# RIKEN-RCCS/EigenExa

Hardware: AMD Instinct MI355X
Metric: eigen_sx full-solve throughput (reference flop model: 4/3 N^3 + D&C GEMM + 2 nvec N^2) (higher is better)
Workload: dtype f64; 1 GPU; N=8192 random symmetric fp64 (counter-based R+R^T, seed 20240807), eigen_sx all eigenpairs, m_forward=64, m_backward=128; parallelism=1 GPU (1x1 grid)

## Files before the change

### eigenexa_amd/csrc/api.hip

```cpp
#include "eigx_context.h"
#include "eigx_comm.h"
#include "../../include/eigenexa_amd.h"
#include <cstring>

namespace eigx {
Context g_ctx;
}

using namespace eigx;

extern "C" {

int eigx_init(int device) {
  return eigx_init_multi(device, 0, 1, nullptr, 'C');
}

int eigx_get_device_count(void) {
  int ndev = 0;
  if (hipGetDeviceCount(&ndev) != hipSuccess) { (void)hipGetLastError(); return 0; }
  return ndev;
}

int eigx_get_rccl_unique_id(void* out128) {
  return comm_get_unique_id(out128);
// ... 160 lines not shown
  const int Px = x_procs, Py = y_procs;
  const int mb = m_backward > 0 ? m_backward : 128;
  const int n1 = ceil_div(n, Px);
  const int n2 = ceil_div(n, Py);
  int lnx;
  int64_t lny;
  if (mode == 'M' || mode == 'm') {
    lnx = n1; lny = n2;
  } else if (mode == 'L' || mode == 'l') {
    lnx = ceil_div(n1, 32) * 32; lny = n2;
  } else {
    lnx = ceil_div(n1, 64) * 64 + 32;
    if (lnx < n1 + 64) lnx += 64;
    const int NB = mb > 64 ? mb : 64;
    int64_t nmz = (int64_t)ceil_div(n1, NB) * NB + 1;
    const int64_t nmz2 = (int64_t)ceil_div(ceil_div(n, NB), Px) * NB;
    if (nmz2 > nmz) nmz = nmz2;
    int64_t nmw = (int64_t)ceil_div(n2, NB) * NB + 1;
    const int64_t nmw2 = (int64_t)ceil_div(ceil_div(n, NB), Py) * NB;
    if (nmw2 > nmw) nmw = nmw2;
    nmz += NB; nmw += NB;
    const int64_t big = nmz > lnx ? nmz : lnx;
    lny = ceil_div64(big * nmw, lnx);
    if (lny < n2) lny = n2;
    lnx = hbm_ld(lnx);
  }
  {
    const int P = Px * Py;
    const int nf = ceil_div(n, P);
    const int64_t nx0 = (int64_t)nf * (P / Px), ny0 = (int64_t)nf * (P / Py);
    if (nx0 > lnx) lnx = (int)nx0;
    if (ny0 > lny) lny = ny0;
  }
  const int pmin = Px < Py ? Px : Py;
  const int64_t side = ceil_div64(ceil_div(n, pmin), 64) * 64;
  if ((side * side >= ((int64_t)1 << 31) || lny >= ((int64_t)1 << 31)) && !(getenv("EIGX_ALLOW_64BIT"))) {
    *nx = -1; *ny = -1;
    return EIGX_ERR_TOO_LARGE;
  }
  *nx = lnx;
  *ny = (int)lny;
  return EIGX_OK;
}

int eigx_get_matdims(int n, int* nx, int* ny, int m_forward, int m_backward, char mode) {
  if (!g_ctx.initialized) return EIGX_ERR_NOT_INITIALIZED;
  return eigx_matdims_for_grid(n, g_ctx.grid.Px, g_ctx.grid.Py, m_forward, m_backward, mode, nx, ny);
}

int64_t eigx_memory_internal(int n, int lda, int ldz, int m_forward, int m_backward) {
  if (!g_ctx.initialized) return -1;
  return solver_workspace_bytes(g_ctx, n, lda, ldz, m_forward, m_backward);
}

int64_t eigx_held_bytes(void) {
  if (!g_ctx.initialized) return -1;
  int64_t t = 0;
  for (const auto& kv : g_ctx.pool.bufs) t += (int64_t)kv.second.bytes;
  return t + comm_held_bytes(g_ctx);
}

int64_t eigx_held_bytes_named(const char* prefix) {
  if (!g_ctx.initialized || !prefix) return -1;
  const std::string pre(prefix);
  int64_t t = 0;
  for (const auto& kv : g_ctx.pool.bufs)
    if (kv.first.compare(0, pre.size(), pre) == 0) t += (int64_t)kv.second.bytes;
  return t;
}

int eigx_get_timers(double* out16) {
  if (!out16) return EIGX_ERR_BAD_ARG;
  for (int i = 0; i < 16; ++i) out16[i] = g_ctx.timers[i];
  return EIGX_OK;
}

int eigx_profile(int stride) {
  if (!g_ctx.initialized) return EIGX_ERR_NOT_INITIALIZED;
  g_ctx.prof_stride = stride > 0 ? stride : 0;
  g_ctx.prof_used = 0;
  g_ctx.prof_kind.clear();
  g_ctx.prof_units.clear();
  return EIGX_OK;
}

int eigx_profile_read(double* out6) {
  if (!g_ctx.initialized) return EIGX_ERR_NOT_INITIALIZED;
  if (!out6) return EIGX_ERR_BAD_ARG;
  EIGX_HIP_CHECK(hipSetDevice(g_ctx.device));
  EIGX_HIP_CHECK(hipStreamSynchronize(g_ctx.stream));
  for (int q = 0; q < 6; ++q) out6[q] = 0.0;
  for (size_t q = 0; q < g_ctx.prof_kind.size(); ++q) {
    float ms = 0.f;
    EIGX_HIP_CHECK(hipEventElapsedTime(&ms, g_ctx.prof_ev[2 * q], g_ctx.prof_ev[2 * q + 1]));
    if (g_ctx.prof_kind[q] > 1) continue;
    const int k = g_ctx.prof_kind[q] ? 3 : 0;
    out6[k + 0] += 1.0;
    out6[k + 1] += g_ctx.prof_units[q];
    out6[k + 2] += 1e-3 * ms;
  }
  return EIGX_OK;
}

int eigx_profile_read_kinds(double* out, int nkinds) {
  if (!g_ctx.initialized) return EIGX_ERR_NOT_INITIALIZED;
  if (!out || nkinds < 1) return EIGX_ERR_BAD_ARG;
  EIGX_HIP_CHECK(hipSetDevice(g_ctx.device));
  EIGX_HIP_CHECK(hipStreamSynchronize(g_ctx.stream));
  for (int q = 0; q < 3 * nkinds; ++q) out[q] = 0.0;
  for (size_t q = 0; q < g_ctx.prof_kind.size(); ++q) {
    const int k = g_ctx.prof_kind[q];
    if (k < 0 || k >= nkinds) continue;
    float ms = 0.f;
    EIGX_HIP_CHECK(hipEventElapsedTime(&ms, g_ctx.prof_ev[2 * q], g_ctx.prof_ev[2 * q + 1]));
    out[3 * k + 0] += 1.0;
    out[3 * k + 1] += g_ctx.prof_units[q];
    out[3 * k + 2] += 1e-3 * ms;
  }
  return EIGX_OK;
}

int eigx_device_synchronize(void) {
  if (!g_ctx.initialized) return EIGX_ERR_NOT_INITIALIZED;
  EIGX_HIP_CHECK(hipSetDevice(g_ctx.device));
  EIGX_HIP_CHECK(hipDeviceSynchronize());
  return EIGX_OK;
}

void* eigx_malloc_dev(int64_t bytes) {
  if (!g_ctx.initialized) return nullptr;
  void* p = nullptr;
  if (hipMalloc(&p, (size_t)bytes) != hipSuccess) return nullptr;
  return p;
}
int eigx_free_dev(void* p) {
  if (p) EIGX_HIP_CHECK(hipFree(p));
  return EIGX_OK;
}
int eigx_memcpy_h2d(void* dst, const void* src, int64_t bytes) {
  EIGX_HIP_CHECK(hipMemcpy(dst, src, (size_t)bytes, hipMemcpyHostToDevice));
  return EIGX_OK;
}
int eigx_memcpy_d2h(void* dst, const void* src, int64_t bytes) {
  EIGX_HIP_CHECK(hipMemcpy(dst, src, (size_t)bytes, hipMemcpyDeviceToHost));
  return EIGX_OK;
}

int eigx_tune(int key, int value) {
  if (key == 0) return set_gemm_variant(value);
  if (key == 1) return set_bisect_threads(value);
  if (key == 2) return set_bt_q(value);
  if (key == 3 || key == 4 || key == 5 || key == 10 || key == 11) return set_reduce_knob(key, value);
  if (key == 12) return (value >= 0 && value <= 2) ? set_reduce_knob(key, value) : -1;
  if (key == 6) return set_gemm_cstream(value);
  if (key == 7) return value > 0 ? set_reduce_knob(key, value) : -1;
  if (key == 8) return set_dc_chunk(value);
  if (key == 9) return comm_set_bounce(value);
  if (key == 15) return set_dc_pipe(value);
  if (key == 16) return set_dc_batch(value);
  if (key == 17 || key == 18 || key == 19) return set_range_knob(key, value);
  if (key == 20) return set_tri_nb(value);
  if (key == 21) return set_batch_nmax(value);
  if (key == 22) return set_hbatch_nmax(value);
  if (key == 23) return set_gbatch_nmax(value);
  if (key == 24) return set_hgbatch_nmax(value);
  if (key == 25) return set_gemm_latec_kmax(value);
  if (key == 26) return set_batch_range_route(value);
  if (key == 27) return set_batch_range_accept(value);
  return -1;
}

int eigx_dgemm_dev(char opa, char opb, int m, int n, int k, double alpha, const double* a, int lda,
                   const double* b, int ldb, double beta, double* c, int ldc, int tri_upper) {
  if (!g_ctx.initialized) return EIGX_ERR_NOT_INITIALIZED;
  EIGX_HIP_CHECK(hipStreamSynchronize(nullptr));
  dgemm_dev(g_ctx.stream, opa, opb, m, n, k, alpha, a, lda, b, ldb, beta, c, ldc, tri_upper ? 1 : 0,
            &g_ctx.grid);
  EIGX_HIP_CHECK(hipStreamSynchronize(g_ctx.stream));
  return EIGX_OK;
}

int eigx_dgemm_gather_dev(char opa, char opb, int m, int n, int k, double alpha, const double* a, int lda,
                          const double* b, int ldb, double beta, double* c, int ldc, const int* kmap_a,
                          const int* kmap_b) {
  if (!g_ctx.initialized) return EIGX_ERR_NOT_INITIALIZED;
  EIGX_HIP_CHECK(hipStreamSynchronize(nullptr));
  dgemm_dev(g_ctx.stream, opa, opb, m, n, k, alpha, a, lda, b, ldb, beta, c, ldc, 0, nullptr, kmap_a, nullptr, 1, 0,
            0, 0, 1, 0, 0, 0, 1, 0, kmap_b);
  EIGX_HIP_CHECK(hipStreamSynchronize(g_ctx.stream));
  return EIGX_OK;
}

}
```

### eigenexa_amd/csrc/band_reduce.hip

```cpp
#include "eigx_context.h"
#include "eigx_comm.h"
#include "../../include/eigenexa_amd.h"
#include <algorithm>
#include <chrono>
#include <cstring>
#include <type_traits>

#pragma clang fp contract(on)

namespace eigx {

namespace {

static inline int pd_rows_for(int toprows) { int r = ((toprows + 3) / 4 + 63) / 64 * 64; return r < 512 ? 512 : r; }
#ifdef EIGX_STAMPS
#define EIGX_ABL(bit) (R.abl & (bit))
#define EIGX_STAMP(slot) do { if (R.dbg && threadIdx.x == 0 && stamp_me) { \
  const unsigned long long _t = __builtin_amdgcn_s_memtime(); atomicAdd(&R.dbg[slot], _t - stamp_prev); stamp_prev = _t; } } while (0)
#define EIGX_STAMP_INIT const bool stamp_me = (bid == nblocks / 2); unsigned long long stamp_prev = __builtin_amdgcn_s_memtime(); (void)stamp_me;
#else
#define EIGX_ABL(bit) false
#define EIGX_STAMP(slot) do {} while (0)
#define EIGX_STAMP_INIT
#endif
constexpr int PD_COLS = 16;
constexpr int KA_ROWS = 16;
constexpr int KA_SL = 256 / KA_ROWS;

enum { SC_SA = 0, SC_BETA_A = 1, SC_SB = 2, SC_BETA_B = 3, SC_COUNT = 8 };

struct RedArgs {
  double* A; int lda; int n;
  double* UW; int ldp; int m;
  double* X;
  double* YR; double* YC;
  double* KD;
  double* SP;
  int sp_packed;
  int kd_compact;
  double* GP;
  double* sc;
  double* d; double* e; int lde;
  int maxseg, maxrs, maxchunk, gp2_off, kdab_off;
  int P, me;
  float invP;
  int Px, Py, px, py, row_major;
  int nxs, nys;
  const double* MSG;
  int msg_stride;
  size_t ypar_stride; int ysrc_stride;
  const double* XW;
  int xmsg_stride, nown;
  size_t xpar_stride;
  const double* PAN; int ldpan;
  const double* zero16;
  int abl;
  int stamp_i;
  unsigned long long* dbg;
};

struct SymvGeom { int L, T, nt; };

int g_ka_fit = 1;
int g_ka_loads = 2;
int g_ka_wgs = 256;
int g_symv_t128 = 4500, g_symv_t256 = 40000;
int g_symv_nt = 9000;
int g_symv_unc = 9000;
}

int set_reduce_knob(int key, int v) {
  int* t = key == 3 ? &g_symv_t128 : key == 4 ? &g_symv_t256 : key == 5 ? &g_symv_nt : key == 7 ? &g_ka_wgs
         : key == 10 ? &g_ka_fit : key == 11 ? &g_symv_unc : key == 12 ? &g_ka_loads : nullptr;
  if (!t) return -1;
  const int old = *t;
  *t = v;
  return old;
}

namespace {

inline SymvGeom symv_geom(int L) {
  SymvGeom g;
  g.L = L;
  g.T = (L <= g_symv_t128) ? 128 : (L <= g_symv_t256 ? 256 : 512);
  g.nt = (L + g.T - 1) / g.T;
  return g;
}

typedef double d2v_t __attribute__((ext_vector_type(2)));
template <bool NT>
__device__ __forceinline__ double2 ld2(const double* p) {
  const d2v_t v = NT ? __builtin_nontemporal_load(reinterpret_cast<const d2v_t*>(p)) : *reinterpret_cast<const d2v_t*>(p);
  return make_double2(v.x, v.y);
}

template <int CTRL>
__device__ __forceinline__ double dpp_add(double v) {
  const int lo = __double2loint(v), hi = __double2hiint(v);
  const int lo2 = __builtin_amdgcn_update_dpp(0, lo, CTRL, 0xf, 0xf, true);
  const int hi2 = __builtin_amdgcn_update_dpp(0, hi, CTRL, 0xf, 0xf, true);
  return v + __hiloint2double(hi2, lo2);
}

template <int CTRL>
__device__ __forceinline__ double dpp_mov(double v) {
  const int lo2 = __builtin_amdgcn_update_dpp(0, __double2loint(v), CTRL, 0xf, 0xf, true);
  const int hi2 = __builtin_amdgcn_update_dpp(0, __double2hiint(v), CTRL, 0xf, 0xf, true);
  return __hiloint2double(hi2, lo2);
}

__device__ __forceinline__ double swapadd32(double a, double b) {
  const auto lo = __builtin_amdgcn_permlane32_swap(__double2loint(a), __double2loint(b), false, false);
  const auto hi = __builtin_amdgcn_permlane32_swap(__double2hiint(a), __double2hiint(b), false, false);
  return __hiloint2double(hi[0], lo[0]) + __hiloint2double(hi[1], lo[1]);
}
__device__ __forceinline__ double swapadd16(double a, double b) {
  const auto lo = __builtin_amdgcn_permlane16_swap(__double2loint(a), __double2loint(b), false, false);
  const auto hi = __builtin_amdgcn_permlane16_swap(__double2hiint(a), __double2hiint(b), false, false);
  return __hiloint2double(hi[0], lo[0]) + __hiloint2double(hi[1], lo[1]);
}

__device__ __forceinline__ double wave_sum(double v) {
  v = dpp_add<0xB1>(v);
  v = dpp_add<0x4E>(v);
  v = dpp_add<0x141>(v);
  v = dpp_add<0x140>(v);
  v = swapadd16(v, v);
  v = swapadd32(v, v);
  return v;
}

template <int K>
__device__ __forceinline__ void block_sum_multi(double (&v)[K], double* red ) {
#pragma unroll
  for (int q = 0; q < K; ++q) v[q] = wave_sum(v[q]);
  __syncthreads();
  if ((threadIdx.x & 63) == 0) {
#pragma unroll
    for (int q = 0; q < K; ++q) red[(threadIdx.x >> 6) * K + q] = v[q];
  }
  __syncthreads();
#pragma unroll
  for (int q = 0; q < K; ++q) v[q] = (red[q] + red[K + q]) + (red[2 * K + q] + red[3 * K + q]);
}

__device__ __forceinline__ double sign_of(double mag, double s) { return s >= 0.0 ? fabs(mag) : -fabs(mag); }

__device__ __forceinline__ double ld_sys(const double* p) { return __hip_atomic_load(p, __ATOMIC_RELAXED, __HIP_MEMORY_SCOPE_SYSTEM); }
__device__ __forceinline__ void st_sys(double* p, double v) { __hip_atomic_store(p, v, __ATOMIC_RELAXED, __HIP_MEMORY_SCOPE_SYSTEM); }

__device__ __forceinline__ double ld_agent(const double* p) { return __hip_atomic_load(p, __ATOMIC_RELAXED, __HIP_MEMORY_SCOPE_AGENT); }
__device__ __forceinline__ void st_agent(double* p, double v) { __hip_atomic_store(p, v, __ATOMIC_RELAXED, __HIP_MEMORY_SCOPE_AGENT); }

struct KAArgs {
  int has_prev;
  int iprev;
  int Lprev;
  int kprev;
  int nchunk_prev;
  int ncols;
  int i;
  int L;
  int k;
  int rows;
  int nt_prev, lgT_prev;
  int par;
  int pan_c0;
  StepWait wait;
  int nchunk_ab;
  int xpar;
  unsigned long long xepoch;
  int G;
};

template <int NB>
__device__ __forceinline__ const double* mg_partial(const RedArgs& R, int par, int t, int r, int& stride) {
  int qx, qy, off;
  if (t < R.Py) { qx = r % R.Px; qy = t; off = r / R.Px; stride = R.nxs; }
  else { qx = t - R.Py; qy = r % R.Py; off = NB * R.nxs + r / R.Py; stride = R.nys; }
  const int src = R.row_major ? qx * R.Py + qy : qx + qy * R.Px;
  return R.MSG + (size_t)par * R.ypar_stride + (size_t)src * R.ysrc_stride + off;
}

__device__ __forceinline__ void own_of(const RedArgs& R, int r, int& src, int& idx) {
  const int g = r >> 4;
  const int q = (int)(((float)g + 0.5f) * R.invP);
  src = g - q * R.P;
  idx = (q << 4) | (r & 15);
}
static_assert(KA_ROWS == 16, "own_of assumes groups of 16 rows");
__device__ __forceinline__ int own_row(const RedArgs& R, int o) { return (((o >> 4) * R.P + R.me) << 4) | (o & 15); }
template <bool MG>
__device__ __forceinline__ double xget(const RedArgs& R, int xpar, int v, int r) {
  if (!MG) return R.X[(size_t)v * R.ldp + r];
  int s_, o_;
  own_of(R, r, s_, o_);
  return ld_sys(R.XW + (size_t)xpar * R.xpar_stride + (size_t)s_ * R.xmsg_stride + (size_t)v * R.nown + o_);
}
__device__ __forceinline__ void step_wait_fused(const StepWait& W, bool first_block) {
  const int tid = threadIdx.x;
  if (tid < W.n) {
    const unsigned long long* f = W.flag + (W.epoch & 1) * EIGX_MAXP + tid;
    const long long t0 = wall_clock64();
    if (__hip_atomic_load(W.err, __ATOMIC_RELAXED, __HIP_MEMORY_SCOPE_SYSTEM) == 0) {
      while (__hip_atomic_load(f, __ATOMIC_RELAXED, __HIP_MEMORY_SCOPE_SYSTEM) < W.epoch) {
        for (int z = 0; z < W.naps; ++z) __builtin_amdgcn_s_sleep(2);
        if (__hip_atomic_load(W.err, __ATOMIC_RELAXED, __HIP_MEMORY_SCOPE_SYSTEM) != 0) break;
        if (wall_clock64() - t0 > W.limit_ticks) {
          __hip_atomic_store(W.err, 2, __ATOMIC_RELAXED, __HIP_MEMORY_SCOPE_SYSTEM);
          break;
        }
      }
    }
    if (first_block && tid == 0) atomicAdd(W.ticks, (unsigned long long)(wall_clock64() - t0));
  }
  __syncthreads();
}

template <int NB, bool MG, bool LG, int RPBT, int SPBT, int KBT, int PWT = 0, bool SPKT = false>
__device__ __forceinline__ void ka_body(const RedArgs& R, const KAArgs& S, const StepPeers* XPp, const int bid, const int nblocks) {
  constexpr int PW = MG ? 0 : PWT;
  constexpr bool SPK = !MG && SPKT;
  constexpr int PWC = PW == 1 ? 64 : 128;
  __shared__ double red[64];
  __shared__ double kd[4][256];
// ... 1193 lines not shown
        }
      }
    }
    if (rb == RB - 1) {
      double fin[NV];
#pragma unroll
      for (int a = 0; a < NV; ++a) {
        double v4[4], v2[2], v1;
        const bool hi8 = lane & 8;
#pragma unroll
        for (int j = 0; j < 4; ++j) v4[j] = swapadd32(yc[a][j], yc[a][j + 4]);
#pragma unroll
        for (int j = 0; j < 2; ++j) v2[j] = swapadd16(v4[j], v4[j + 2]);
        {
          const double keep = hi8 ? v2[1] : v2[0];
          const double send = hi8 ? v2[0] : v2[1];
          v1 = keep + dpp_mov<0x128>(send);
        }
        v1 = dpp_add<0xB1>(v1);
        v1 = dpp_add<0x4E>(v1);
        v1 = dpp_add<0x141>(v1);
        fin[a] = v1;
      }
      if ((lane & 7) == 0) {
        const int j = ((lane >> 5) & 1) * 4 + ((lane >> 4) & 1) * 2 + ((lane >> 3) & 1);
        const int c = col0 + tc0 + j;
        if (c < Lc) {
#pragma unroll
          for (int a = 0; a < NV; ++a) {
            R.YC[((size_t)ty * NV + a) * ldp + c] = fin[a];
          }
          const double ua = ucs[tc0 + j];
          sp[0] += ua * fin[0];
          if (NV == 2) { sp[1] += ua * fin[NV - 1]; sp[2] += ucs[(NV - 1) * T + tc0 + j] * fin[NV - 1]; }
        }
      }
    }
  };

#define EIGX_PIN do { if (UNC) asm volatile("" ::: "memory"); } while (0)
  {
    if (RB == 1) {
      for (int g = 0; g < NG; g += 2) {
        load8(av1, g + 1, 0);
        EIGX_PIN;
        compute8(av0, g, IC<0>());
        load8_next(av0, g + 2, g + 1, g + 2 < NG);
        EIGX_PIN;
        compute8(av1, g + 1, IC<0>());
      }
    } else if (RB == 2) {
      const int ng = B.ng;
#pragma unroll 1
      for (int g = 0; g < ng; ++g) {
        load8(av1, g, 1);
        EIGX_PIN;
        compute8(av0, g, IC<0>());
        load8_next(av0, g + 1, g, g + 1 < ng);
        EIGX_PIN;
        compute8(av1, g, IC<(RB > 1 ? 1 : 0)>());
      }
    } else {
      const int ng = B.ng;
#pragma unroll 1
      for (int g = 0; g < ng; ++g) {
        load8(av1, g, 1);
        EIGX_PIN;
        compute8(av0, g, IC<0>());
        load8(av0, g, 2);
        EIGX_PIN;
        compute8(av1, g, IC<(RB > 1 ? 1 : 0)>());
        load8(av1, g, 3);
        EIGX_PIN;
        compute8(av0, g, IC<(RB > 2 ? 2 : 0)>());
        load8_next(av0, g + 1, g, g + 1 < ng);
        EIGX_PIN;
        compute8(av1, g, IC<(RB > 3 ? 3 : 0)>());
      }
    }
  }

  EIGX_STAMP(10);
  if (EIGX_ABL(256)) {
    if (yr[0][0][0] == 1.2345678) R.SP[0] = yr[0][0][1] + yr[NV - 1][RB - 1][0];
    return;
  }
#pragma unroll
  for (int rb = 0; rb < RB; ++rb) {
#pragma unroll
    for (int a = 0; a < NV; ++a) {
      double* dst = yrs + ((size_t)wave * NV + a) * T + rb * 128 + lane * 2;
      dst[0] = yr[a][rb][0];
      dst[1] = yr[a][rb][1];
    }
    sp[0] += ux[0][rb][0] * yr[0][rb][0] + ux[0][rb][1] * yr[0][rb][1];
    if (NV == 2) {
      sp[1] += ux[0][rb][0] * yr[NV - 1][rb][0] + ux[0][rb][1] * yr[NV - 1][rb][1];
      sp[2] += ux[NV - 1][rb][0] * yr[NV - 1][rb][0] + ux[NV - 1][rb][1] * yr[NV - 1][rb][1];
    }
  }
  __syncthreads();
  for (int rep_ = 0; rep_ < (EIGX_ABL(4096) ? 2 : 1); ++rep_) {
  if (rep_) {
    __syncthreads();
#pragma unroll
    for (int rb = 0; rb < RB; ++rb)
#pragma unroll
      for (int a = 0; a < NV; ++a) {
        double* dst = yrs + ((size_t)wave * NV + a) * T + rb * 128 + lane * 2;
        dst[0] = yr[a][rb][0];
        dst[1] = yr[a][rb][1];
      }
    __syncthreads();
  }
  if (!EIGX_ABL(1024))
  for (int t = tid; t < T; t += 256) {
    const int r = row0 + t;
    if (r < Lr) {
#pragma unroll
      for (int a = 0; a < NV; ++a) {
        const double s = (yrs[((size_t)0 * NV + a) * T + t] + yrs[((size_t)1 * NV + a) * T + t]) +
                         (yrs[((size_t)2 * NV + a) * T + t] + yrs[((size_t)3 * NV + a) * T + t]);
        R.YR[((size_t)tx * NV + a) * ldp + r] = s;
      }
    }
  }
  }
  if (EIGX_ABL(8192)) {
    double s2[3] = {sp[0], sp[1], sp[2]};
    block_sum_multi<3>(s2, red);
    __syncthreads();
    if (s2[0] == 1.2345678) sp[0] = s2[1];
  }
  if (!EIGX_ABL(512)) block_sum_multi<3>(sp, red);
  if (tid == 0) {
    const size_t w = (!MG && R.sp_packed) ? (size_t)bid : (size_t)ty * R.maxseg + tx;
    R.SP[w * 3 + 0] = sp[0]; R.SP[w * 3 + 1] = sp[1]; R.SP[w * 3 + 2] = sp[2];
  }
  EIGX_STAMP(11);
#ifdef EIGX_STAMPS
  if (R.dbg && threadIdx.x == 0 && stamp_me) atomicAdd(&R.dbg[15], 1ull);
  if (MG && R.dbg && threadIdx.x == 0 && B.i == R.stamp_i) {
    const unsigned long long t_ = (unsigned long long)wall_clock64();
    atomicMax(&R.dbg[3908], t_); atomicMax(&R.dbg[3909], ~t_); atomicAdd(&R.dbg[3910], 1ull);
  }
#endif
}

template <int NV, int RB, bool NTL, bool MG, bool UNC>
__global__ __launch_bounds__(256) void symv_kernel(RedArgs R, KBArgs B) {
  symv_body<NV, RB, NTL, MG, UNC>(R, B, blockIdx.x, gridDim.x);
}

struct MGStep { int nkl, nka; StepPeers xpeers; };
template <int NV, int RB, bool NTL, bool UNC>
__global__ __launch_bounds__(256) void mg_step_kernel(RedArgs R, KLArgs KL, KAArgs S, KBArgs B, MGStep M) {
  int bid = blockIdx.x;
#ifdef EIGX_STAMPS
  if (R.dbg && bid == 0 && threadIdx.x == 0 && M.nkl > 0 && M.nka > 0 && (int)gridDim.x > M.nkl + M.nka) {
    const unsigned long long t = (unsigned long long)wall_clock64();
    const unsigned long long prev = R.dbg[20];
    if (prev != 0 && t - prev < 100000ull) { atomicAdd(&R.dbg[21], t - prev); atomicAdd(&R.dbg[24], 1ull); }
    __hip_atomic_store(&R.dbg[20], t, __ATOMIC_RELAXED, __HIP_MEMORY_SCOPE_AGENT);
  }
#endif
  if (bid < M.nkl) { kl_body<NV>(R, KL, bid, M.nkl); return; }
  bid -= M.nkl;
  if (bid < M.nka) { ka_body<NV, true, false, 1, 8, 8>(R, S, &M.xpeers, bid, M.nka); return; }
  bid -= M.nka;
  symv_body<NV, RB, NTL, true, UNC>(R, B, bid, (int)gridDim.x - M.nkl - M.nka);
}

__global__ void compact_panel_kernel(const double* __restrict__ UW, int ldp, int m, int nrl, int ncl, int Px, int px,
                                     int Py, int py, double* __restrict__ UWr, int ldr, double* __restrict__ UWc, int ldc) {
  const int k = blockIdx.y;
  const double* rsrc = UW + (size_t)k * ldp;
  const double* csrc = UW + (size_t)(k + m) * ldp;
  for (int l = blockIdx.x * blockDim.x + threadIdx.x; l < (nrl > ncl ? nrl : ncl); l += gridDim.x * blockDim.x) {
    if (l < nrl) UWr[(size_t)k * ldr + l] = rsrc[(size_t)l * Px + px];
    if (l < ncl) UWc[(size_t)k * ldc + l] = csrc[(size_t)l * Py + py];
  }
}

__global__ void pack_panel_kernel(const double* __restrict__ A, int lda, int lj0, int mloc, int nrl, int nxs,
                                  double* __restrict__ send) {
  const int ljr = blockIdx.y;
  if (ljr >= mloc) return;
  for (int li = blockIdx.x * blockDim.x + threadIdx.x; li < nrl; li += gridDim.x * blockDim.x)
    send[(size_t)ljr * nxs + li] = A[(size_t)(lj0 + ljr) * lda + li];
}
__global__ void unpack_panel_kernel(const double* __restrict__ recv, size_t count, int nxs, int clo, int chi, int toprows,
                                    int Px, int Py, int row_major, double* __restrict__ PAN, int ldpan) {
  const int c = clo + blockIdx.y;
  if (c > chi) return;
  const int qy = c % Py;
  const int lj0 = (clo - qy + Py - 1) / Py;
  const int ljr = c / Py - lj0;
  for (int r = blockIdx.x * blockDim.x + threadIdx.x; r < toprows; r += gridDim.x * blockDim.x) {
    const int qx = r % Px;
    const int src = row_major ? qx * Py + qy : qx + qy * Px;
    PAN[(size_t)(c - clo) * ldpan + r] = ld_sys(recv + (size_t)src * count + (size_t)ljr * nxs + r / Px);
  }
}

template <int NB>
__global__ void mg_wcopy_kernel(RedArgs R, int xpar, int wk, int rows, StepWait W) {
  if (W.n > 0) step_wait_fused(W, blockIdx.x == 0);
  double* Wp = R.UW + (size_t)R.ldp * R.m;
  for (int r = blockIdx.x * blockDim.x + threadIdx.x; r < rows; r += gridDim.x * blockDim.x) {
    int s_, o_;
    own_of(R, r, s_, o_);
    const double* xm = R.XW + (size_t)xpar * R.xpar_stride + (size_t)s_ * R.xmsg_stride + o_;
    Wp[(size_t)wk * R.ldp + r] = ld_sys(xm + 2 * (size_t)R.nown);
    if (NB == 2) Wp[(size_t)(wk + 1) * R.ldp + r] = ld_sys(xm + 3 * (size_t)R.nown);
  }
}
template <int NB>
__global__ void mg_tail_kernel(RedArgs R, int xpar, int i, int ncols, StepWait W) {
  if (W.n > 0) step_wait_fused(W, blockIdx.x == 0);
  if (threadIdx.x == 0 && ncols > 0) {
    R.d[i] = xget<true>(R, xpar, 0, i);
    if (ncols > 1) { R.e[i] = xget<true>(R, xpar, 0, i - 1); R.d[i - 1] = xget<true>(R, xpar, 1, i - 1); }
  }
}

inline double wall_seconds() { return std::chrono::duration<double>(std::chrono::steady_clock::now().time_since_epoch()).count(); }
inline StepWait no_wait() { return StepWait{nullptr, nullptr, nullptr, 0, 0, 0, 1}; }
inline void clear_panel(const RedArgs& R, hipStream_t st) {
  hipLaunchKernelGGL(fill_kernel, dim3(1024), dim3(256), 0, st, R.UW, (size_t)R.ldp * R.m * 3, 0.0);
}

template <int NB>
RedArgs reduce_setup(Context& ctx, int n, double* A, int lda, double* d, double* e, int lde, int m) {
  m = std::min(std::max(m, NB), 256);
  if (NB == 2 && (m & 1)) ++m;
  const int ldp = pad_ld((n + 127) / 128 * 128 + 128);
  const Grid& G = ctx.grid;
  const bool mg = G.nranks > 1;
  RedArgs R;
  R.A = A; R.lda = lda; R.n = n; R.ldp = ldp; R.m = m;
  R.d = d; R.e = e; R.lde = lde;
  R.P = G.nranks; R.me = G.rank; R.invP = 1.0f / (float)G.nranks;
  R.Px = G.Px; R.Py = G.Py; R.px = G.px; R.py = G.py; R.row_major = G.row_major;
  R.nxs = (ceil_div(n, G.Px) + 7) / 8 * 8; R.nys = (ceil_div(n, G.Py) + 7) / 8 * 8;
  R.msg_stride = NB * (R.nxs + R.nys) + 8 + 2 * NB * m;
  R.ypar_stride = (size_t)G.nranks * R.msg_stride; R.ysrc_stride = R.msg_stride;
  R.nown = ceil_div(ceil_div(n, KA_ROWS), G.nranks) * KA_ROWS;
  R.xmsg_stride = 4 * R.nown + 8;
  R.xpar_stride = (size_t)G.nranks * R.xmsg_stride;
  R.MSG = nullptr; R.XW = nullptr; R.PAN = nullptr; R.ldpan = ldp;
  int maxseg = 0;
  if (mg) maxseg = ceil_div(R.nxs > R.nys ? R.nxs : R.nys, 128) + 1;
  else for (int L = n; L >= 1; --L) maxseg = std::max(maxseg, symv_geom(L).nt);
  maxseg += 1;
  R.maxseg = maxseg; R.maxrs = maxseg; R.maxchunk = 4 + 1;
  R.UW = ctx.pool.get_t<double>("red.UW", (size_t)ldp * (m * 3 + 128));
  R.X = ctx.pool.get_t<double>("red.X", (size_t)ldp * 3);
  if (!mg) {
    const int nslot = (maxseg + 2 > 162) ? maxseg + 2 : 162;
    R.YC = ctx.pool.get_t<double>("red.Y", (size_t)nslot * NB * ldp);
    R.YR = R.YC + (size_t)NB * ldp;
    R.kdab_off = R.maxchunk * 2 * NB * m;
    R.KD = ctx.pool.get_t<double>("red.KD", (size_t)R.kdab_off + R.maxchunk + 8 + 512);
  } else {
    R.YR = ctx.pool.get_t<double>("red.YR", (size_t)maxseg * NB * ldp);
    R.YC = ctx.pool.get_t<double>("red.YC", (size_t)R.maxrs * NB * ldp);
    const int maxchunk2 = 12;
    R.kdab_off = maxchunk2 * 2 * NB * m;
    R.KD = ctx.pool.get_t<double>("red.KD2", (size_t)R.kdab_off + 4 * G.nranks + 4 + 8 + 512);
  }
  R.SP = ctx.pool.get_t<double>("red.SP", (size_t)(maxseg * maxseg) * 3 + 8);
  R.sp_packed = (!mg && g_ka_loads >= 1) ? 1 : 0;
  R.kd_compact = (!mg && g_ka_loads >= 2) ? 1 : 0;
  R.gp2_off = 0;
  R.GP = ctx.pool.get_t<double>("red.GP", (size_t)((n + KA_ROWS - 1) / KA_ROWS + 2) * 3 + 8);
  R.sc = ctx.pool.get_t<double>("red.sc", SC_COUNT + 8);
  R.zero16 = R.sc + SC_COUNT;
  R.dbg = nullptr; R.abl = 0; R.stamp_i = -1;
#ifdef EIGX_STAMPS
  R.abl = getenv("EIGX_ABL") ? atoi(getenv("EIGX_ABL")) : 0;
  R.stamp_i = getenv("EIGX_STAMP_I") ? atoi(getenv("EIGX_STAMP_I")) : -1;
  R.dbg = ctx.pool.get_t<unsigned long long>("red.dbg", 4096);
  EIGX_HIP_CHECK(hipMemsetAsync(R.dbg, 0, 4096 * sizeof(unsigned long long), ctx.stream));
#endif
  clear_panel(R, ctx.stream);
  hipLaunchKernelGGL(fill_kernel, dim3(8), dim3(256), 0, ctx.stream, e, (size_t)lde * NB, 0.0);
  hipLaunchKernelGGL(fill_kernel, dim3(1), dim3(64), 0, ctx.stream, R.sc, (size_t)SC_COUNT + 8, 0.0);
  hipLaunchKernelGGL(fill_kernel, dim3(16), dim3(256), 0, ctx.stream, R.SP, (size_t)(maxseg * maxseg) * 3 + 8, 0.0);
  return R;
}

struct RedCounters {
  long n_symv = 0, n_k1 = 0; double symv_bytes = 0.0, k1_flops = 0.0;
  bool sampled(const Context& ctx) const { return ctx.prof_stride > 0 && (n_symv % ctx.prof_stride) == 0; }
  void step(int L) { symv_bytes += 8.0 * ((double)L * (L + 1) / 2); ++n_symv; }
  void panel(int nr, int m) { k1_flops += 2.0 * (double)nr * nr * m; ++n_k1; }
  void write(Context& ctx) const { ctx.timers[6] = (double)n_k1; ctx.timers[7] = k1_flops; ctx.timers[9] = (double)n_symv; ctx.timers[10] = symv_bytes; }
};
inline KAArgs ka_first_args() { KAArgs S{}; S.lgT_prev = 7; S.G = 1; S.wait = no_wait(); return S; }
template <int NB>
inline int ka_step_args(KAArgs& S, int i, int k) {
  const int L = i - NB + 1;
  S.ncols = (L >= 1) ? NB : (i >= 0 ? (i + 1 < NB ? i + 1 : NB) : 0);
  S.i = i; S.L = (L >= 1) ? L : 0; S.k = k;
  S.rows = (S.has_prev && S.iprev + 1 > i + 1) ? S.iprev + 1 : i + 1;
  return L;
}
template <int NB>
inline void step_done(KAArgs& S, RedCounters& C, int& i, int& k, int L, int nt, int T, int nchunk, int nchunk_ab) {
  C.step(L);
  S.has_prev = 1; S.iprev = i; S.Lprev = L; S.kprev = k; S.nchunk_prev = nchunk; S.nchunk_ab = nchunk_ab;
  S.nt_prev = nt; S.lgT_prev = (T == 128) ? 7 : (T == 256 ? 8 : 9);
  k += NB;
  i -= NB;
}
template <int NB>
inline bool panel_full(int k, int m, int i) { return k >= m && i - NB + 1 >= 1; }
inline void panel_restart(const RedArgs& R, RedCounters& C, KAArgs& S, int& k, int nr, hipStream_t st) {
  C.panel(nr, R.m); clear_panel(R, st); S.has_prev = 0; k = 0;
}
inline KAArgs ka_close_args(const KAArgs& S, int i, int k) { KAArgs F = S; F.ncols = 0; F.i = i; F.L = 0; F.k = k; F.rows = S.iprev + 1; return F; }
inline KBArgs kb_step_args(int i, int L, int k) {
  KBArgs B;
  B.i = i; B.L = L; B.k = k;
  B.ncg = (k + PD_COLS - 1) / PD_COLS; B.toprows = i + 1; B.pdr = pd_rows_for(B.toprows);
  B.nown_L = 0; B.npd_s = 0; B.pdr_s = 0; B.wk = -1; B.xpar = 0; B.xwait = no_wait();
  B.Lr = L; B.Lc = L; B.ntc = 0; B.nty_last = 0; B.slope = 0; B.c1 = 0;
  return B;
}
inline void trace_enqueue(double t_begin, hipStream_t st) {
  if (!getenv("EIGX_TRACE_ENQUEUE")) return;
  const double te = wall_seconds();
  EIGX_HIP_CHECK(hipStreamSynchronize(st));
  fprintf(stderr, "[eigx] reduction: enqueue loop %.1f ms, then %.1f ms until the stream drained\n", (te - t_begin) * 1e3, (wall_seconds() - te) * 1e3);
}
inline void stamps_report(const RedArgs& R, int NB, hipStream_t st) {
#ifdef EIGX_STAMPS
  const bool mg = R.P > 1;
  unsigned long long h[32];
  EIGX_HIP_CHECK(hipStreamSynchronize(st));
  EIGX_HIP_CHECK(hipMemcpy(h, R.dbg, sizeof(h), hipMemcpyDeviceToHost));
  if (mg && h[24]) fprintf(stderr, "[eigx stamps] step launch timeline (100-MHz clock, averages over %llu full launches, from workgroup 0's entry): Y flags "
                           "raised at %.2f us, X flags at %.2f us, next launch's workgroup 0 enters at %.2f us\n", h[24], 0.01 * h[22] / h[24],
                           0.01 * h[23] / h[24], 0.01 * h[21] / h[24]);
  if (R.stamp_i >= 0 && mg) {
    std::vector<unsigned long long> big(4096);
    EIGX_HIP_CHECK(hipMemcpy(big.data(), R.dbg, 4096 * sizeof(unsigned long long), hipMemcpyDeviceToHost));
    unsigned long long t0 = ~0ull; int nw = 0, nk = 0;
    for (int b = 0; b < 256; ++b) if (big[3136 + b]) { ++nk; if (big[3136 + b] < t0) t0 = big[3136 + b]; }
    for (int b = 0; b < 1024; ++b) if (big[64 + b]) { ++nw; if (big[64 + b] < t0) t0 = big[64 + b]; }
    double mk[3] = {0, 0, 0}, mx[3] = {0, 0, 0};
    for (int b = 0; b < nk; ++b) for (int q = 0; q < 3; ++q) { const double v = 0.01 * (big[3136 + 256 * q + b] - t0); if (v > mk[q]) mk[q] = v; }
    for (int b = 0; b < nw; ++b) for (int q = 0; q < 3; ++q) { const double v = 0.01 * (big[64 + 1024 * q + b] - t0); if (v > mx[q]) mx[q] = v; }
    fprintf(stderr, "[eigx stamps] step with top column %d, us after the launch's first workgroup: kl role (%d workgroups) latest entry %.2f, partial sums in %.2f, "
            "stores drained %.2f | ka role (%d) latest entry %.2f, Y seen %.2f, pushes issued %.2f; count complete %.2f, X flags stored %.2f | mat-vec role "
            "(%llu tiles): X seen first %.2f last %.2f, tile ends first %.2f last %.2f\n", R.stamp_i, nk, mk[0], mk[1], mk[2], nw, mx[0], mx[1], mx[2],
            0.01 * (big[3904] - t0), 0.01 * (big[3905] - t0), big[3910], 0.01 * (~big[3906] - t0), 0.01 * (big[3907] - t0), 0.01 * (~big[3909] - t0),
            0.01 * (big[3908] - t0));
  }
  if (h[30]) fprintf(stderr, "[eigx stamps] K_A workgroup in the middle: %.2f us of wall clock per launch, %.0f s_memtime ticks: %.0f MHz\n",
                     0.01 * h[30] / h[7], (double)h[31] / h[7], (double)h[31] / (0.01 * h[30]));
  if (mg && h[24]) fprintf(stderr, "[eigx stamps] ka role, workgroup in the middle: enters at %.2f us, sees the Y flags at %.2f, has issued its pushes at %.2f; "
                           "the watcher sees the count complete at %.2f us\n", 0.01 * h[26] / h[7], 0.01 * h[27] / h[7], 0.01 * h[28] / h[7], 0.01 * h[29] / h[14]);
  if (mg) fprintf(stderr, "[eigx stamps] K_A several GPUs: wait %.0f | to the end of the pushes %.0f, drain + barrier %.0f | last arriver (from its previous stamp "
                  "to the flag store) %.0f x %llu\n", (double)h[5] / h[7], (double)h[6] / h[7], (double)h[12] / h[7], (double)h[13] / (h[14] ? h[14] : 1), h[14]);
  fprintf(stderr, "[eigx stamps] NB=%d n=%d K_A launches %llu: avg cycles issue %.0f consume %.0f reduce %.0f rows %.0f tail %.0f | SYMV %llu: "
          "entry %.0f scalars %.0f stream %.0f tail %.0f\n", NB, R.n, h[7], (double)h[0] / h[7], (double)h[1] / h[7], (double)h[2] / h[7],
          (double)h[3] / h[7], (double)h[4] / h[7], h[15], (double)h[8] / (h[15] ? h[15] : 1), (double)h[9] / (h[15] ? h[15] : 1),
          (double)h[10] / (h[15] ? h[15] : 1), (double)h[11] / (h[15] ? h[15] : 1));
#endif
}

inline int ka_grid_one_gpu(int rows, int& G) {
  const int ng = (rows + KA_ROWS - 1) / KA_ROWS;
  G = (ng > 2 * g_ka_wgs) ? (ng + g_ka_wgs - 1) / g_ka_wgs : 1;
  const int nwg = (ng + G - 1) / G;
  return nwg > 0 ? nwg : 1;
}

template <int NB>
void launch_ka(hipStream_t st, int nwg, const RedArgs& R, const KAArgs& K) {
  const bool fit = g_ka_fit != 0;
  const int nslot = fit ? K.nt_prev + 1 : 1 << 30, ntp = fit ? K.nt_prev : 1 << 30;
  const int ntl = fit ? K.nt_prev * (K.nt_prev + 1) / 2 : 1 << 30;
  const int kk = fit ? (K.has_prev ? K.kprev : K.k) : 1 << 30;
  const int pw = (fit && R.kd_compact) ? (R.m <= 64 ? 1 : R.m <= 128 ? 2 : 0) : 0;
  auto go = [&](auto rpb, auto spb, auto spk) {
    auto go_kb = [&](auto kb, auto pwc) {
      constexpr int RPB = decltype(rpb)::value, SPB = decltype(spb)::value, KB = decltype(kb)::value, PW = decltype(pwc)::value;
      constexpr bool SPK = decltype(spk)::value;
      if (K.G > 1) hipLaunchKernelGGL((ka_kernel<NB, false, true, RPB, SPB, KB, PW, SPK>), dim3(nwg), dim3(256), 0, st, R, K);
      else hipLaunchKernelGGL((ka_kernel<NB, false, false, RPB, SPB, KB, PW, SPK>), dim3(nwg), dim3(256), 0, st, R, K);
    };
    auto go_pw = [&](auto kb) {
      if constexpr (decltype(spk)::value) {
        if constexpr (decltype(kb)::value <= 4) {
          if (pw == 1) return go_kb(kb, IC<1>{});
        }
        if (pw == 2) return go_kb(kb, IC<2>{});
      }
      go_kb(kb, IC<0>{});
    };
    if (kk <= 2 * KA_SL) go_pw(IC<2>{}); else if (kk <= 4 * KA_SL) go_pw(IC<4>{}); else go_pw(IC<8>{});
  };
  if (R.sp_packed) {
    const std::true_type pk{};
    if (nslot <= 1 * KA_SL && ntl <= 256) go(IC<1>{}, IC<1>{}, pk);
    else if (nslot <= 2 * KA_SL && ntl <= 256) go(IC<2>{}, IC<1>{}, pk);
    else if (nslot <= 2 * KA_SL && ntl <= 512) go(IC<2>{}, IC<2>{}, pk);
    else if (nslot <= 3 * KA_SL && ntl <= 768) go(IC<3>{}, IC<3>{}, pk);
    else if (nslot <= 3 * KA_SL && ntl <= 1024) go(IC<3>{}, IC<4>{}, pk);
    else if (nslot <= 3 * KA_SL) go(IC<3>{}, IC<8>{}, pk);
    else if (nslot <= 5 * KA_SL) go(IC<5>{}, IC<8>{}, pk);
    else go(IC<10>{}, IC<8>{}, pk);
    return;
  }
  const std::false_type fl{};
  if (nslot <= 1 * KA_SL && ntp <= 15) go(IC<1>{}, IC<2>{}, fl);
  else if (nslot <= 2 * KA_SL && ntp <= 31) go(IC<2>{}, IC<4>{}, fl);
  else if (nslot <= 3 * KA_SL) go(IC<3>{}, IC<8>{}, fl);
  else if (nslot <= 5 * KA_SL) go(IC<5>{}, IC<8>{}, fl);
  else go(IC<10>{}, IC<8>{}, fl);
}

template <class Go>
void symv_variant(int T, bool nt_loads, bool unc, Go&& go) {
  auto u = [&](auto rb, auto ntl) { if (unc) go(rb, ntl, std::true_type{}); else go(rb, ntl, std::false_type{}); };
  if (T == 128) u(IC<1>{}, std::false_type{});
  else if (T == 256 && !nt_loads) u(IC<2>{}, std::false_type{});
  else if (T == 256) u(IC<2>{}, std::true_type{});
  else if (!nt_loads) u(IC<4>{}, std::false_type{});
  else u(IC<4>{}, std::true_type{});
}
template <int NB>
void launch_symv(hipStream_t st, int gx, const RedArgs& R, const KBArgs& B, int T, bool nt_loads, bool unc) {
  symv_variant(T, nt_loads, unc, [&](auto rb, auto ntl, auto un) {
    hipLaunchKernelGGL((symv_kernel<NB, decltype(rb)::value, decltype(ntl)::value, false, decltype(un)::value>), dim3(gx), dim3(256), 0, st, R, B);
  });
}

template <int NB>
void reduce_one_gpu(Context& ctx, const RedArgs& R, RedCounters& C) {
  const hipStream_t st = ctx.stream;
  const int m = R.m, ldp = R.ldp;
  const double t_begin = wall_seconds();
  KAArgs S = ka_first_args();
  int k = 0, i = R.n - 1;
  while (true) {
    const int L = ka_step_args<NB>(S, i, k);
    const int nb_ka = ka_grid_one_gpu(S.rows, S.G);
    if (S.rows > 0 && (S.has_prev || S.ncols > 0)) launch_ka<NB>(st, nb_ka, R, S);
    if (L < 1) break;
    KBArgs B = kb_step_args(i, L, k);
    const SymvGeom g = symv_geom(L);
    B.npd = (B.toprows + B.pdr - 1) / B.pdr; B.ngp = nb_ka; B.nt = g.nt; B.ng = g.T / 32;
    const int gx = g.nt * (g.nt + 1) / 2 + B.npd * (B.ncg + 1);
    const bool prof = C.sampled(ctx);
    if (prof) ctx.prof_begin(0, 8.0 * ((double)L * (L + 1) / 2), st);
    launch_symv<NB>(st, gx, R, B, g.T, L > g_symv_nt, L <= g_symv_unc);
    if (prof) ctx.prof_end(st);
    step_done<NB>(S, C, i, k, L, g.nt, g.T, B.npd, B.npd);
    if (panel_full<NB>(k, m, i)) {
      KAArgs F = ka_close_args(S, i, k);
      const int nb_kf = ka_grid_one_gpu(F.rows, F.G);
      launch_ka<NB>(st, nb_kf, R, F);
      const int nr = i + 1;
      if (ctx.prof_stride > 0) ctx.prof_begin(1, 2.0 * (double)nr * nr * m, st);
      dgemm_dev(st, 'N', 'T', nr, nr, 2 * m, -1.0, R.UW, ldp, R.UW + (size_t)ldp * m, ldp, 1.0, R.A, R.lda, 1);
      if (ctx.prof_stride > 0) ctx.prof_end(st);
      panel_restart(R, C, S, k, nr, st);
    }
  }
  trace_enqueue(t_begin, st);
}

template <int NB>
void launch_mg_step(hipStream_t st, int gx, const RedArgs& R, const KLArgs& KL, const KAArgs& S, const KBArgs& B,
                    const MGStep& M, int symv_T, bool nt_loads, bool unc) {
  if (symv_T == 0) hipLaunchKernelGGL((mg_step_kernel<NB, 1, false, true>), dim3(gx), dim3(256), 0, st, R, KL, S, B, M);
  else symv_variant(symv_T, nt_loads, unc, [&](auto rb, auto ntl, auto un) {
    hipLaunchKernelGGL((mg_step_kernel<NB, decltype(rb)::value, decltype(ntl)::value, decltype(un)::value>), dim3(gx), dim3(256), 0, st,
                       R, KL, S, B, M);
  });
}

inline int mg_step_geom(KBArgs& B, const Grid& G, int L, int& ntiles) {
  const int gfull = L / KA_ROWS, rem = L % KA_ROWS;
  B.nown_L = local_count(gfull, G.nranks, G.rank) * KA_ROWS + ((rem > 0 && gfull % G.nranks == G.rank) ? rem : 0);
  B.pdr = std::max(512, ((B.nown_L + 7) / 8 + 63) / 64 * 64);
  B.npd = (B.nown_L + B.pdr - 1) / B.pdr;
  B.pdr_s = std::max(512, ((B.toprows + 4 * G.nranks - 1) / (4 * G.nranks) + 63) / 64 * 64);
  B.npd_s = (B.toprows + B.pdr_s - 1) / B.pdr_s;
  B.ngp = G.nranks;
  B.Lr = local_count(L, G.Px, G.px); B.Lc = local_count(L, G.Py, G.py);
  const double leq = sqrt((double)(B.Lr > 1 ? B.Lr : 1) * (double)(B.Lc > 1 ? B.Lc : 1));
  const int T = (leq <= g_symv_t128) ? 128 : (leq <= g_symv_t256 ? 256 : 512);
  B.ntc = B.nt = ceil_div(B.Lc, T); B.ng = T / 32;
  ntiles = B.nty_last = B.ntc > 0 ? mg_nty(B.ntc - 1, T, B.Lc, G.Px, G.px, G.Py, G.py) : 0;
  for (int tx = 0; tx + 1 < B.ntc; ++tx) ntiles += mg_nty(tx, T, B.Lc, G.Px, G.px, G.Py, G.py);
  if (G.Py % G.Px == 0) { B.slope = G.Py / G.Px; B.c1 = (int)(((long)(T - 1) * G.Py + G.py - G.px) / ((long)G.Px * T)) + 1; }
  return T;
}

template <int NB>
void reduce_multi_rank(Context& ctx, RedArgs& R, RedCounters& C) {
  const hipStream_t st = ctx.stream;
  const Grid& G = ctx.grid;
  const int n = R.n, m = R.m, ldp = R.ldp;
  StepPeers peers, xpeers;
  R.MSG = comm_step_window(ctx, 0, (size_t)R.msg_stride, &peers); R.ysrc_stride = (int)peers.src_stride;
  R.XW = comm_step_window(ctx, 1, (size_t)R.xmsg_stride, &xpeers);
  unsigned long long epoch = comm_step_epoch_base(ctx, 0, (unsigned long long)(n / NB + 2));
  unsigned long long xepoch = comm_step_epoch_base(ctx, 1, (unsigned long long)(n / NB + n / m + 8));
  const int mloc_max = ceil_div(m + NB, G.Py) + 1;
  const size_t pan_count = (size_t)mloc_max * R.nxs;
  const int ldr = pad_ld(R.nxs + 2), ldc = pad_ld(R.nys + 2);
  PeerBuf* panr = comm_buffer(ctx, "red.panr", (size_t)G.nranks * pan_count * sizeof(double));
  double* pan = ctx.pool.get_t<double>("red.pan", (size_t)ldp * (m + NB));
  double* pan_send = ctx.pool.get_t<double>("red.pansend", pan_count);
  double* UWr = ctx.pool.get_t<double>("red.UWr", (size_t)ldr * 2 * m);
  double* UWc = ctx.pool.get_t<double>("red.UWc", (size_t)ldc * 2 * m);
  R.PAN = pan;
  EIGX_HIP_CHECK(hipMemsetAsync(pan_send, 0, pan_count * sizeof(double), st));
  auto panel_lo = [&](int itop) { const int clo = itop - m + 1; return clo <= NB ? 0 : clo; };
  auto gather_panel = [&](int clo, int chi, hipStream_t s, CommChannel ch) {
    const int toprows = chi + 1;
    const int nxc = (ceil_div(toprows, G.Px) + 7) / 8 * 8;
    const size_t cnt = (size_t)mloc_max * nxc;
    const int lj0 = (clo - G.py + G.Py - 1) / G.Py, lj1 = chi >= G.py ? (chi - G.py) / G.Py : -1;
    const int mloc = lj1 - lj0 + 1;
    const int nrl = local_count(toprows, G.Px, G.px);
    if (mloc > 0 && nrl > 0)
      hipLaunchKernelGGL(pack_panel_kernel, dim3(ceil_div(nrl, 256) < 64 ? ceil_div(nrl, 256) : 64, mloc), dim3(256), 0, s,
                         (const double*)R.A, R.lda, lj0, mloc, nrl, nxc, pan_send);
    comm_exchange(ctx, COMM_WORLD, pan_send, 0, panr, 0, cnt, s, ch);
    hipLaunchKernelGGL(unpack_panel_kernel, dim3(ceil_div(toprows, 256) < 64 ? ceil_div(toprows, 256) : 64, chi - clo + 1),
                       dim3(256), 0, s, (const double*)panr->local, cnt, nxc, clo, chi, toprows, G.Px, G.Py,
                       G.row_major, pan, ldp);
  };
  const double t_begin = wall_seconds();
  KAArgs S = ka_first_args();
  const StepWait none = no_wait();
  const bool fuse_wait = comm_step_wait_fused(ctx);
  const bool step_coll = comm_step_collective(ctx);
  const int step_fence = (getenv("EIGX_STEP_FENCE") && atoi(getenv("EIGX_STEP_FENCE")) != 0) ? 1 : 0;
  int naps_ka = 1, naps_x = 2;
  if (const char* e = getenv("EIGX_SPIN_NAPS")) { if (sscanf(e, "%d,%d", &naps_ka, &naps_x) < 2) naps_x = naps_ka; }
  MGStep MS{}; MS.xpeers = xpeers;
  KBArgs Bnone{}; Bnone.xwait = none;
  const KLArgs KLnone{};
  auto launch_roles = [&](int nkl, const KLArgs& KLa, int nka, const KAArgs& Ka, int nsymv, const KBArgs& Ba, int symv_T, bool nt_loads, bool unc) {
    MGStep M = MS; M.nkl = nkl; M.nka = nka;
    if (nkl + nka + nsymv > 0) launch_mg_step<NB>(st, nkl + nka + nsymv, R, KLa, Ka, Ba, M, symv_T, nt_loads, unc);
  };
  int wk_last = -1, last_ka_i = -1, last_ka_ncols = 0;
  KLArgs KLp = KLnone;
  int nkl_p = 0;
  bool prof_step = false;
  auto ka_grid = [&](int rows) { const int own = local_count(ceil_div(rows, KA_ROWS), G.nranks, G.rank); return own > 0 ? own : 1; };
  auto wait_kernel = [&](int which, unsigned long long ep, int prof_kind) {
    if (prof_kind >= 0) ctx.prof_begin(prof_kind, 0.0, st);
    comm_step_wait(ctx, which, ep, st);
    if (prof_kind >= 0) ctx.prof_end(st);
  };
  auto ka_begin = [&](KAArgs& K) {
    ++xepoch;
    K.xpar = (int)(xepoch & 1); K.xepoch = xepoch;
    wk_last = K.has_prev ? K.kprev : -1; last_ka_i = K.i; last_ka_ncols = K.ncols;
    K.wait = (fuse_wait && K.has_prev) ? comm_step_wait_args(ctx, 0, epoch) : none;
    K.wait.naps = naps_ka;
  };
  auto ka_launch = [&](int nwg, const KAArgs& K, bool prof_it) {
    if (fuse_wait) { launch_roles(nkl_p, KLp, nwg, K, 0, Bnone, 0, false, true); nkl_p = 0; return; }
    if (K.has_prev && !step_coll) wait_kernel(0, epoch, prof_it ? 3 : -1);
    if (prof_it) ctx.prof_begin(4, 0.0, st);
    launch_roles(0, KLnone, nwg, K, 0, Bnone, 0, false, true);
    if (step_coll) comm_step_allgather(ctx, 1, xpeers.slot[0], K.xpar, st);
    if (prof_it) ctx.prof_end(st);
  };
  auto x_wait = [&](int prof_kind) -> StepWait {
    if (step_coll) return none;
    if (fuse_wait) { StepWait w = comm_step_wait_args(ctx, 1, xepoch); w.naps = naps_x; return w; }
    wait_kernel(1, xepoch, prof_kind);
    return none;
  };
  int k = 0, i = n - 1;
  S.pan_c0 = panel_lo(n - 1);
  gather_panel(S.pan_c0, n - 1, st, CH_BULK);
  while (true) {
    const int L = ka_step_args<NB>(S, i, k);
    const int nb_ka = ka_grid(S.rows);
    const bool need_ka = S.rows > 0 && (S.has_prev || S.ncols > 0);
    const bool ka_held = need_ka && fuse_wait;
    if (need_ka) ka_begin(S);
    if (need_ka && !fuse_wait) ka_launch(nb_ka, S, prof_step);
    if (L < 1) { if (ka_held) ka_launch(nb_ka, S, false); break; }
    KBArgs B = kb_step_args(i, L, k);
    int ntiles;
    const int T = mg_step_geom(B, G, L, ntiles);
    B.wk = wk_last; B.xpar = (int)(xepoch & 1);
    B.xwait = x_wait(prof_step ? 5 : -1); prof_step = false;
    const int gx = ntiles + B.npd * B.ncg + B.npd_s;
    const bool prof = C.sampled(ctx);
    if (prof) ctx.prof_begin(0, 8.0 * ((double)L * (L + 1) / 2) / R.P, st);
    const double leq = sqrt((double)B.Lr * B.Lc);
    if (ka_held) launch_roles(nkl_p, KLp, nb_ka, S, gx, B, T, leq > g_symv_nt, leq <= g_symv_unc);
    else launch_roles(0, KLnone, 0, S, gx, B, T, leq > g_symv_nt, leq <= g_symv_unc);
    nkl_p = 0;
    if (prof) ctx.prof_end(st);
    KLArgs KL{};
    ++epoch;
    KL.L = L; KL.Lr = B.Lr; KL.Lc = B.Lc; KL.T = T; KL.ntc = B.ntc;
    KL.nbr = ceil_div(B.Lr > 0 ? B.Lr : 1, KL_ROWS);
    KL.par = (int)(epoch & 1); KL.epoch = epoch; KL.peers = peers;
    KL.kd2 = R.KD; KL.npd2 = B.npd; KL.kfill = k; KL.fence = step_fence;
    for (int tx = 0; tx < B.ntc; ++tx) { const int c_ = mg_nty(tx, T, B.Lc, G.Px, G.px, G.Py, G.py); if (c_ > KL.ntr) KL.ntr = c_; }
    const int nkl = KL.nbr + ceil_div(B.Lc > 0 ? B.Lc : 1, KL_ROWS) + 2 * NB + 1;
    if (fuse_wait) { KLp = KL; nkl_p = nkl; }
    else {
      if (prof) ctx.prof_begin(2, 8.0 * R.msg_stride, st);
      launch_roles(nkl, KL, 0, S, 0, Bnone, 0, false, true);
      if (step_coll) comm_step_allgather(ctx, 0, peers.slot[0], KL.par, st);
      if (prof) ctx.prof_end(st);
// ... 65 lines not shown
```

Before: 19410 GFLOP/s.

## Fold panel-close KA into next step and fuse UW zero-fill into SYMV

At a panel boundary the single-GPU band reduction now launches the next step's KA kernel in place of the separate close KA, and skips it at the top of the next iteration. The UW buffer reset that panel_restart did is moved into extra blocks appended to the next SYMV launch, and those blocks leave the rows of active slot columns untouched. The aim is to remove one kernel launch and one fill launch per panel, at the cost of relying on the KA step args being valid across the trailing GEMM update. A new tuning knob (key 13) selects the path and defaults to the fully fused mode.

```diff
diff --git a/eigenexa_amd/csrc/api.hip b/eigenexa_amd/csrc/api.hip
--- a/eigenexa_amd/csrc/api.hip
+++ b/eigenexa_amd/csrc/api.hip
@@ -336,6 +336,7 @@
   if (key == 2) return set_bt_q(value);
   if (key == 3 || key == 4 || key == 5 || key == 10 || key == 11) return set_reduce_knob(key, value);
   if (key == 12) return (value >= 0 && value <= 2) ? set_reduce_knob(key, value) : -1;
+  if (key == 13) return (value >= 0 && value <= 2) ? set_reduce_knob(key, value) : -1;
   if (key == 6) return set_gemm_cstream(value);
   if (key == 7) return value > 0 ? set_reduce_knob(key, value) : -1;
   if (key == 8) return set_dc_chunk(value);
diff --git a/eigenexa_amd/csrc/band_reduce.hip b/eigenexa_amd/csrc/band_reduce.hip
--- a/eigenexa_amd/csrc/band_reduce.hip
+++ b/eigenexa_amd/csrc/band_reduce.hip
@@ -67,11 +67,12 @@
 int g_symv_t128 = 4500, g_symv_t256 = 40000;
 int g_symv_nt = 9000;
 int g_symv_unc = 9000;
+int g_panel_boundary = 2;
 }
 
 int set_reduce_knob(int key, int v) {
   int* t = key == 3 ? &g_symv_t128 : key == 4 ? &g_symv_t256 : key == 5 ? &g_symv_nt : key == 7 ? &g_ka_wgs
-         : key == 10 ? &g_ka_fit : key == 11 ? &g_symv_unc : key == 12 ? &g_ka_loads : nullptr;
+         : key == 10 ? &g_ka_fit : key == 11 ? &g_symv_unc : key == 12 ? &g_ka_loads : key == 13 ? &g_panel_boundary : nullptr;
   if (!t) return -1;
   const int old = *t;
   *t = v;
@@ -1571,6 +1572,18 @@
   symv_body<NV, RB, NTL, MG, UNC>(R, B, blockIdx.x, gridDim.x);
 }
 
+template <int NV, int RB, bool NTL, bool UNC>
+__global__ __launch_bounds__(256) void symv_kernel_with_fill(RedArgs R, KBArgs B, int nsymv) {
+  if ((int)blockIdx.x >= nsymv) {
+    const int c = (int)blockIdx.x - nsymv;
+    const bool slot = (c >= B.k && c < B.k + NV) || (c >= 2 * R.m + B.k && c < 2 * R.m + B.k + NV);
+    double* col = R.UW + (size_t)c * R.ldp;
+    for (int r = (slot ? B.toprows : 0) + (int)threadIdx.x; r < R.ldp; r += 256) col[r] = 0.0;
+    return;
+  }
+  symv_body<NV, RB, NTL, false, UNC>(R, B, blockIdx.x, nsymv);
+}
+
 struct MGStep { int nkl, nka; StepPeers xpeers; };
 template <int NV, int RB, bool NTL, bool UNC>
 __global__ __launch_bounds__(256) void mg_step_kernel(RedArgs R, KLArgs KL, KAArgs S, KBArgs B, MGStep M) {
@@ -1852,9 +1865,12 @@
   else u(IC<4>{}, std::true_type{});
 }
 template <int NB>
-void launch_symv(hipStream_t st, int gx, const RedArgs& R, const KBArgs& B, int T, bool nt_loads, bool unc) {
+void launch_symv(hipStream_t st, int gx, const RedArgs& R, const KBArgs& B, int T, bool nt_loads, bool unc, bool with_fill = false) {
   symv_variant(T, nt_loads, unc, [&](auto rb, auto ntl, auto un) {
-    hipLaunchKernelGGL((symv_kernel<NB, decltype(rb)::value, decltype(ntl)::value, false, decltype(un)::value>), dim3(gx), dim3(256), 0, st, R, B);
+    if (with_fill)
+      hipLaunchKernelGGL((symv_kernel_with_fill<NB, decltype(rb)::value, decltype(ntl)::value, decltype(un)::value>), dim3(gx + 3 * R.m), dim3(256), 0, st, R, B, gx);
+    else
+      hipLaunchKernelGGL((symv_kernel<NB, decltype(rb)::value, decltype(ntl)::value, false, decltype(un)::value>), dim3(gx), dim3(256), 0, st, R, B);
   });
 }
 
@@ -1863,12 +1879,19 @@
   const hipStream_t st = ctx.stream;
   const int m = R.m, ldp = R.ldp;
   const double t_begin = wall_seconds();
+  const bool early = g_panel_boundary >= 1, fused_fill = g_panel_boundary >= 2;
   KAArgs S = ka_first_args();
   int k = 0, i = R.n - 1;
+  int L = 0, nb_ka = 0;
+  bool formed = false;
+  bool fill_due = false;
   while (true) {
-    const int L = ka_step_args<NB>(S, i, k);
-    const int nb_ka = ka_grid_one_gpu(S.rows, S.G);
-    if (S.rows > 0 && (S.has_prev || S.ncols > 0)) launch_ka<NB>(st, nb_ka, R, S);
+    if (!formed) {
+      L = ka_step_args<NB>(S, i, k);
+      nb_ka = ka_grid_one_gpu(S.rows, S.G);
+      if (S.rows > 0 && (S.has_prev || S.ncols > 0)) launch_ka<NB>(st, nb_ka, R, S);
+    }
+    formed = false;
     if (L < 1) break;
     KBArgs B = kb_step_args(i, L, k);
     const SymvGeom g = symv_geom(L);
@@ -1876,18 +1899,27 @@
     const int gx = g.nt * (g.nt + 1) / 2 + B.npd * (B.ncg + 1);
     const bool prof = C.sampled(ctx);
     if (prof) ctx.prof_begin(0, 8.0 * ((double)L * (L + 1) / 2), st);
-    launch_symv<NB>(st, gx, R, B, g.T, L > g_symv_nt, L <= g_symv_unc);
+    launch_symv<NB>(st, gx, R, B, g.T, L > g_symv_nt, L <= g_symv_unc, fill_due);
+    fill_due = false;
     if (prof) ctx.prof_end(st);
     step_done<NB>(S, C, i, k, L, g.nt, g.T, B.npd, B.npd);
     if (panel_full<NB>(k, m, i)) {
-      KAArgs F = ka_close_args(S, i, k);
-      const int nb_kf = ka_grid_one_gpu(F.rows, F.G);
-      launch_ka<NB>(st, nb_kf, R, F);
+      if (early) {
+        L = ka_step_args<NB>(S, i, k);
+        nb_ka = ka_grid_one_gpu(S.rows, S.G);
+        launch_ka<NB>(st, nb_ka, R, S);
+        formed = true;
+      } else {
+        KAArgs F = ka_close_args(S, i, k);
+        const int nb_kf = ka_grid_one_gpu(F.rows, F.G);
+        launch_ka<NB>(st, nb_kf, R, F);
+      }
       const int nr = i + 1;
       if (ctx.prof_stride > 0) ctx.prof_begin(1, 2.0 * (double)nr * nr * m, st);
       dgemm_dev(st, 'N', 'T', nr, nr, 2 * m, -1.0, R.UW, ldp, R.UW + (size_t)ldp * m, ldp, 1.0, R.A, R.lda, 1);
       if (ctx.prof_stride > 0) ctx.prof_end(st);
-      panel_restart(R, C, S, k, nr, st);
+      if (fused_fill) { C.panel(nr, m); S.has_prev = 0; k = 0; fill_due = true; }
+      else panel_restart(R, C, S, k, nr, st);
     }
   }
   trace_enqueue(t_begin, st);
```

New measurement: 19500 GFLOP/s, median of 6. Within noise of the previous version (+0.5%).
